# jesusbriales/dvo_slam

Hardware: AMD Instinct MI355X
Metric: frame-pairs/s (640x480, 4-level GN align) (higher is better)
Workload: dtype f32

## Files before the change

### dvo_slam_amd/capi.py

```python
from __future__ import annotations

import ctypes as C
import os

import numpy as np

from . import _build

MAX_LEVELS = 8
TERMINATION = {0: "IterationsExceeded", 1: "IncrementTooSmall", 2: "LogLikelihoodDecreased", 3: "TooFewConstraints",
               -1: "Unset"}

EXPORTS = [
    "dvo_amd_abi_version", "dvo_amd_build_id", "dvo_amd_status_string", "dvo_amd_last_error", "dvo_amd_device_count",
    "dvo_amd_default_config", "dvo_amd_context_create", "dvo_amd_context_destroy", "dvo_amd_configure",
    "dvo_amd_get_config", "dvo_amd_pyramid_create", "dvo_amd_pyramid_create_from_device", "dvo_amd_pyramid_retain",
    "dvo_amd_pyramid_release", "dvo_amd_pyramid_levels", "dvo_amd_pyramid_timestamp", "dvo_amd_pyramid_level_info",
    "dvo_amd_pyramid_download_plane", "dvo_amd_pyramid_select", "dvo_amd_match", "dvo_amd_match_batch",
    "dvo_amd_residuals", "dvo_amd_error_image", "dvo_amd_kernel_timing", "dvo_amd_se3_exp", "dvo_amd_se3_log",
    "dvo_amd_solve6", "dvo_amd_bench_residual_pass", "dvo_amd_match_many",
    "dvo_amd_debug_finalize_stamps", "dvo_amd_comm_unique_id", "dvo_amd_comm_create", "dvo_amd_comm_destroy",
    "dvo_amd_match_sharded", "dvo_amd_match_banded", "dvo_amd_context_device", "dvo_amd_debug_combine_bands", "dvo_amd_debug_wire_layout", "dvo_amd_debug_take_wire", "dvo_amd_pyramid_create_raw",
    "dvo_amd_default_validator_stages", "dvo_amd_proposals_for_candidates", "dvo_amd_validate_proposals",
    "dvo_amd_track_frame", "dvo_amd_png_info", "dvo_amd_png_read_bgr8", "dvo_amd_png_read_gray16",
    "dvo_amd_format_trajectory_line", "dvo_amd_debug_tick_log", "dvo_amd_debug_iteration", "dvo_amd_match_selection", "dvo_amd_bench_residual_pass_pairs",
    "dvo_amd_exchange_create", "dvo_amd_exchange_attach", "dvo_amd_exchange_destroy",
    "dvo_amd_match_submit", "dvo_amd_match_wait", "dvo_amd_match_poll", "dvo_amd_debug_next_seq",
    "dvo_amd_set_reciprocal_mode", "dvo_amd_get_reciprocal_mode", "dvo_amd_debug_rcp", "dvo_amd_debug_block_trace",
    "dvo_amd_debug_ll_overflow", "dvo_amd_debug_marker", "dvo_amd_debug_rcp_form", "dvo_amd_debug_weights", "dvo_amd_debug_hw_queue",
    "dvo_amd_debug_level_geometry", "dvo_amd_point_cloud", "dvo_amd_map_cloud", "dvo_amd_voxel_downsample", "dvo_amd_write_pcd",
    "dvo_amd_debug_map_timing", "dvo_amd_default_graph_options", "dvo_amd_optimize_graph", "dvo_amd_graph_marginals", "dvo_amd_debug_graph_timing",
    "dvo_amd_debug_graph_system", "dvo_amd_debug_graph_system_sparse", "dvo_amd_debug_graph_symbolic",
    "dvo_amd_debug_graph_sparse_timing", "dvo_amd_optimize_graphs_batch", "dvo_amd_debug_graph_batch_records",
]


class CConfig(C.Structure):
    _fields_ = [("first_level", C.c_int), ("last_level", C.c_int), ("max_iterations_per_level", C.c_int),
                ("precision", C.c_double), ("mu", C.c_double), ("use_initial_estimate", C.c_int),
                ("intensity_derivative_threshold", C.c_float), ("depth_derivative_threshold", C.c_float),
                ("segment_geometry", C.c_int), ("reserved", C.c_int)]


GEOMETRY_THROUGHPUT, GEOMETRY_LATENCY = 0, 1


class CIterationStats(C.Structure):
    _fields_ = [("id", C.c_int), ("valid_constraints", C.c_int), ("tdist_loglik", C.c_double),
                ("tdist_mean", C.c_double * 2), ("tdist_precision", C.c_double * 4), ("prior_loglik", C.c_double),
                ("increment", C.c_double * 6), ("information", C.c_double * 36), ("has_increment", C.c_int),
                ("reserved", C.c_int), ("estimate", C.c_double * 16), ("initial", C.c_double * 16)]


class CLevelStats(C.Structure):
    _fields_ = [("id", C.c_int), ("max_valid_pixels", C.c_int), ("valid_pixels", C.c_int), ("termination", C.c_int),
                ("n_iterations", C.c_int), ("first_iteration", C.c_int)]
# ... 121 lines not shown
    L.dvo_amd_debug_weights.argtypes = [vp, vp, vp, C.c_int, fp, fp, fp, C.POINTER(CQ7Probe)]
    L.dvo_amd_kernel_timing.argtypes = [vp, C.c_int, dp, C.POINTER(C.c_longlong), C.c_int]
    L.dvo_amd_bench_residual_pass.argtypes = [vp, vp, vp, C.c_int, fp, C.c_int, C.c_int, C.c_int, dp, dp,
                                              C.POINTER(C.c_int)]
    L.dvo_amd_bench_residual_pass_pairs.argtypes = [vp, C.c_int, C.POINTER(vp), C.POINTER(vp), C.c_int, fp, C.c_int, C.c_int, dp, dp,
                                                    C.POINTER(C.c_int)]
    L.dvo_amd_debug_finalize_stamps.argtypes = [vp, C.POINTER(C.c_ulonglong)]
    L.dvo_amd_comm_unique_id.argtypes = [C.POINTER(C.c_ubyte)]
    L.dvo_amd_comm_create.argtypes = [vp, C.POINTER(C.c_ubyte), C.c_int, C.c_int]
    L.dvo_amd_comm_destroy.argtypes = [vp]
    L.dvo_amd_comm_destroy.restype = None
    L.dvo_amd_exchange_create.argtypes = [vp, C.c_int, C.c_int, C.POINTER(C.c_ubyte)]
    L.dvo_amd_exchange_attach.argtypes = [vp, C.POINTER(C.c_ubyte)]
    L.dvo_amd_exchange_destroy.argtypes = [vp]
    L.dvo_amd_exchange_destroy.restype = None
    L.dvo_amd_match_sharded.argtypes = [vp, vp, vp, dp, C.POINTER(CResult)]
    L.dvo_amd_match_banded.argtypes = [vp, vp, vp, dp, C.POINTER(CResult), C.c_int]
    L.dvo_amd_debug_combine_bands.argtypes = [C.c_int, dp, dp]
    L.dvo_amd_debug_block_trace.restype = C.c_longlong
    L.dvo_amd_debug_block_trace.argtypes = [C.c_void_p, C.POINTER(C.c_ulonglong), C.c_longlong]
    L.dvo_amd_debug_wire_layout.argtypes = [C.POINTER(C.c_int), C.POINTER(C.c_int)]
    L.dvo_amd_debug_take_wire.argtypes = [C.POINTER(C.c_uint), C.c_uint, C.c_int, C.POINTER(C.c_uint)]
    L.dvo_amd_debug_next_seq.argtypes = [C.c_uint]
    L.dvo_amd_debug_next_seq.restype = C.c_uint
    L.dvo_amd_point_cloud.argtypes = [vp, vp, C.c_int, dp, vp, C.c_int, vp]
    L.dvo_amd_map_cloud.argtypes = [vp, C.c_int, C.POINTER(vp), dp, C.POINTER(vp), C.POINTER(C.c_int), C.c_float, vp,
                                    C.c_longlong, C.POINTER(CCloudStats)]
    L.dvo_amd_voxel_downsample.argtypes = [vp, C.c_longlong, vp, C.c_float, vp, C.c_longlong, C.POINTER(CCloudStats)]
    L.dvo_amd_write_pcd.argtypes = [C.c_char_p, vp, C.c_longlong, C.c_int, C.c_int]
    L.dvo_amd_debug_map_timing.argtypes = [vp, dp, dp, C.POINTER(C.c_longlong)]
    L.dvo_amd_se3_exp.argtypes = [dp, dp]
    L.dvo_amd_se3_exp.restype = None
    L.dvo_amd_se3_log.argtypes = [dp, dp]
    L.dvo_amd_se3_log.restype = None
    L.dvo_amd_solve6.argtypes = [dp, dp, dp]
    L.dvo_amd_solve6.restype = None
    _lib = L
    return L


def build_id() -> str:
    return lib().dvo_amd_build_id().decode()


def _check(status: int, where: str):
    if status != 0:
# ... 582 lines not shown


def comm_unique_id() -> bytes:
    buf = (C.c_ubyte * 128)()
    _check(lib().dvo_amd_comm_unique_id(buf), "dvo_amd_comm_unique_id")
    return bytes(buf)


def wire_layout():
    a, b = C.c_int(), C.c_int()
    _check(lib().dvo_amd_debug_wire_layout(C.byref(a), C.byref(b)), "wire_layout")
    return a.value, b.value


def take_wire(wire: np.ndarray, tick: int, from_piece: int, record: np.ndarray) -> int:
    up = C.POINTER(C.c_uint)
    assert wire.dtype == np.uint32 and record.dtype == np.uint32 and wire.flags.c_contiguous and record.flags.c_contiguous
    rc = lib().dvo_amd_debug_take_wire(wire.ctypes.data_as(up), tick, from_piece, record.ctypes.data_as(up))
    if rc < 0:
        _check(-rc, "take_wire")
    return rc


def combine_bands(bands) -> np.ndarray:
    b = np.ascontiguousarray(bands, dtype=np.float64)
    out = np.zeros(7)
    dp = C.POINTER(C.c_double)
    _check(lib().dvo_amd_debug_combine_bands(b.shape[0], b.ctypes.data_as(dp), out.ctypes.data_as(dp)), "combine_bands")
    return out
```

### dvo_slam_amd/csrc/dvo_internal.h

```cpp
#pragma once
#include <hip/hip_runtime.h>
#include <rccl/rccl.h>

#include <atomic>
#include <deque>
#include <memory>
#include <mutex>
#include <string>
#include <vector>

#include "../../include/dvo_amd.h"
#include "../../include/dvo_amd_debug.h"
#include "dvo_types.h"
#include "se3.h"

namespace dvo_amd {
namespace host {

extern thread_local std::string g_last_error;
int fail_hip(const char *what, hipError_t e);

#define HIP_TRY(expr)                                                     \
  do {                                                                    \
    hipError_t e_ = (expr);                                               \
// ... 120 lines not shown
  unsigned *x_host_seq = nullptr;
  unsigned x_seq = 0;
  bool x_broken = false;
  ExchangeArgs *x_args_dev = nullptr;
  ncclResult_t (*p_allgather)(const void *, void *, size_t, ncclDataType_t, ncclComm_t, hipStream_t) = nullptr;
  ncclResult_t (*p_comm_destroy)(ncclComm_t) = nullptr;
  unsigned tick_seq = 0;
  RcpTable rcp = {nullptr, 0, 0, nullptr};
  unsigned *rcp_table_dev = nullptr;
  unsigned *rcp_nibbles_dev = nullptr;
  int rcp_unit = 0;
  std::string rcp_form_note;
  int q7_off256 = 0;
  float *dbg_w_dev = nullptr;
  size_t dbg_w_capacity = 0;
  unsigned *ovf_host = nullptr, *ovf_dev = nullptr;
  long long ovf_checks = 0, ovf_hits = 0;
  long long level_steps_at[5] = {18, 70, 1000, 1000, 1LL << 40};
  long long level_steps_at_latency[5] = {250, 4000, 38400, 999999, 1LL << 40};
  int fine_steps = 0;
  int fault_slot_alloc = -1;
  bool fin_stamps = false;
  bool sort_items = true;
  bool fin_priority = true;
  bool small_args = true;
  bool poll = true;
  bool timing = false;
  double timing_ms = 0.0;
  long long timing_launches = 0;
  std::vector<double> tick_log;
  std::vector<double> tick_log_pending;
  std::vector<std::pair<hipEvent_t, hipEvent_t>> events;
  size_t events_used = 0;
  host::MapWorkspace *map_ws = nullptr;
  host::GraphWorkspace *graph_ws = nullptr;
  host::GraphBatchWorkspace *graph_batch_ws = nullptr;
};

namespace dvo_amd {
namespace host {

struct IterCtx {
  int k = 0;
  int buf = 0;
  int steps = 4;
  int n_blocks = 0;
// ... 154 lines not shown
```

### dvo_slam_amd/csrc/dvo_kernels.hip

```cpp
#include <cstddef>
#include <cstdlib>
#include <cstring>
#include <mutex>
#include <vector>

#include "dvo_types.h"

namespace dvo_amd {


#define DVO_HWREG_MODE_FP32_ROUND (1 | (0 << 6) | ((2 - 1) << 11))
#define DVO_OPAQUE(x) asm volatile("" : "+v"(x))
#ifndef DVO_KT_SGPR
#define DVO_KT_SGPR 1
#endif

__device__ __forceinline__ void round_toward_zero() { __builtin_amdgcn_s_setreg(DVO_HWREG_MODE_FP32_ROUND, 3); }
__device__ __forceinline__ void round_to_nearest() { __builtin_amdgcn_s_setreg(DVO_HWREG_MODE_FP32_ROUND, 0); }

__device__ __forceinline__ float mul_legacy(float a, float b) {
  float r;
  asm("v_mul_legacy_f32 %0, %1, %2" : "=v"(r) : "v"(a), "v"(b));
  return r;
}

// ... 830 lines not shown
      unsigned hw, xcc;
      asm volatile("s_getreg_b32 %0, hwreg(HW_REG_HW_ID)" : "=s"(hw));
      asm volatile("s_getreg_b32 %0, hwreg(HW_REG_XCC_ID)" : "=s"(xcc));
      BlockTrace t;
      t.t0 = trace_t0, t.t_first = trace_first, t.t_end = trace_t1;
#ifdef DVO_TRACE_TAIL
      if (bx < rb) {
        const unsigned long long t_spin = trace_clock();
        unsigned long long tail = 0;
        while ((tail = __hip_atomic_load(&trace_tail, __ATOMIC_RELAXED, __HIP_MEMORY_SCOPE_WORKGROUP)) == 0 && trace_clock() - t_spin < 2000) {}
        t.t_first = tail;
      }
#endif
      t.info = (unsigned)(bx < rb ? (it.steps_log2 & 15) : (it.steps_log2 >> 4)) | (bx < rb ? 0u : 16u) | ((unsigned)(d.w / 8) << 8) |
               ((unsigned)(bx < rb ? rb : it.ll_blocks) << 16);
      t.hw = (hw & 0x0fffffffu) | (xcc << 28);
      g_trace[slot] = t;
    }
  }
#endif
}

template <class Args>
__device__ __forceinline__ int tick_locate(const Args &args, int &bx, const unsigned block = blockIdx.x) {
  constexpr int kSlots = (int)(sizeof(args.group_first) / sizeof(args.group_first[0]));
  if (!args.compact) {
    const int rot = args.xcd_rot[blockIdx.y];
    bx = (int)((block & ~7u) | ((block + rot) & 7u));
    return (int)blockIdx.y;
  }
  const int lane = threadIdx.x & (kWave - 1);
  const unsigned g = block >> 3;
  const unsigned first = lane <= args.n_items ? (unsigned)args.group_first[lane < kSlots ? lane : 0] : 0xFFFFFFFFu;
  const int idx = __builtin_amdgcn_readfirstlane(__popcll(__ballot(first <= g)) - 1);
  bx = (int)block - ((int)args.group_first[idx] << 3);
  bx = (bx & ~7) | ((bx + (int)args.xcd_rot[idx]) & 7);
  return idx;
}

template <int ACC, int RCP>
__global__ __launch_bounds__(kBlockThreads, ACC == 0 ? 2 : 4) void k_tick(const TickArgs args) {
  int bx;
  const int idx = tick_locate(args, bx);
  tick_body<ACC, RCP>(args.items[idx], args.rcp, bx);
}

template <int RCP>
__global__ __launch_bounds__(kBlockThreads, 4) void k_tick_small(const TickArgsSmall args) {
  int bx;
  const int idx = tick_locate(args, bx);
  tick_body<1, RCP>(args.items[idx], args.rcp, bx);
}

template <class Args>
__device__ __forceinline__ void q7_tail_wave(const Args &args) {
  const TickItem &it = args.items[blockIdx.x];
  const int lane = threadIdx.x;
  LevelPairDesc d = load_desc(it);
  d.rcp = args.rcp;
  d.rcp_lds = nullptr, d.dbg_w = nullptr;
// ... 166 lines not shown
  bool held;
  LaunchGuard() {
    held = launch_lock_enabled();
    if (held) g_launch_mu.lock();
  }
  ~LaunchGuard() {
    if (held) g_launch_mu.unlock();
  }
};

int acc_mode() {
  static const int m = [] {
    const char *a = getenv("DVO_AMD_ACCUM");
    return (a && (a[0] == 'v' || a[0] == 'V' || a[0] == '0')) ? 0 : 1;
  }();
  return m;
}

typedef void (*TickKernel)(const TickArgs);
static TickKernel pick_tick_kernel(const RcpTable &rcp) {
  return rcp.nibbles ? k_tick<1, 2> : rcp.table ? k_tick<1, 1> : acc_mode() == 0 ? k_tick<0, 0> : k_tick<1, 0>;
}

template <class Args>
static int tick_args_layout_impl(Args &args, int max_blocks) {
  constexpr int kSlots = (int)(sizeof(args.group_first) / sizeof(args.group_first[0]));
  unsigned groups = 0;
  for (int i = 0; i < args.n_items; ++i) {
    args.group_first[i] = (uint16_t)groups;
    groups += ((unsigned)args.items[i].res_blocks + args.items[i].ll_blocks + 7u) >> 3;
  }
  for (int i = args.n_items; i < kSlots; ++i) args.group_first[i] = (uint16_t)groups;
  static const bool rotate = [] {
    const char *e = getenv("DVO_AMD_XCD_ROTATE");
    return !(e && e[0] == '0');
  }();
  long long load[8] = {0, 0, 0, 0, 0, 0, 0, 0};
  for (int i = 0; i < args.n_items; ++i) {
    const TickItem &it = args.items[i];
    const int rb = it.res_blocks, lb = it.ll_blocks;
    const long long w_res = 33 + 21 * item_res_steps(it), w_ll = 40 + 7 * item_ll_steps(it);
    long long phase[8];
    for (int f = 0; f < 8; ++f) {
      const int n_res = (rb >> 3) + (f < (rb & 7) ? 1 : 0);
      const int all = ((rb + lb) >> 3) + (f < ((rb + lb) & 7) ? 1 : 0);
      phase[f] = w_res * n_res + w_ll * (all - n_res);
    }
    int best = 0;
    long long best_max = -1;
    for (int rot = 0; rotate && rot < 8; ++rot) {
      long long mx = 0;
      for (int x = 0; x < 8; ++x) mx = std::max(mx, load[x] + phase[(x + rot) & 7]);
      if (best_max < 0 || mx < best_max) best_max = mx, best = rot;
    }
    args.xcd_rot[i] = (uint8_t)best;
    for (int x = 0; x < 8; ++x) load[x] += phase[(x + best) & 7];
  }
  for (int i = args.n_items; i < (int)(sizeof(args.xcd_rot) / sizeof(args.xcd_rot[0])); ++i) args.xcd_rot[i] = 0;
  const long long grid2d = (long long)((max_blocks + 7) & ~7) * args.n_items;
  static const int mode = [] {
    const char *e = getenv("DVO_AMD_COMPACT_GRID");
    return e ? (e[0] == '0' ? 0 : 1) : 2;
  }();
  args.compact = groups > 0 && groups < 65536 && (mode == 1 || (mode == 2 && 2ll * 8 * groups < grid2d)) ? 1 : 0;
  return (int)(groups * 8);
}
int tick_args_layout(TickArgs &args, int max_blocks) { return tick_args_layout_impl(args, max_blocks); }
int tick_args_layout(TickArgsSmall &args, int max_blocks) { return tick_args_layout_impl(args, max_blocks); }

hipError_t launch_tick_small(const TickArgsSmall &args, int max_blocks, hipStream_t stream, hipEvent_t t_start, hipEvent_t t_stop) {
  if (acc_mode() != 1) return hipErrorNotSupported;
  if (args.n_items <= 0 || max_blocks <= 0) return hipSuccess;
  LaunchGuard guard;
  dim3 grid((unsigned)((max_blocks + 7) & ~7), (unsigned)args.n_items, 1);
  if (args.compact) grid = dim3((unsigned)args.group_first[args.n_items] * 8u, 1, 1);
  if (t_start && t_stop) {
    void *kargs[] = {const_cast<TickArgsSmall *>(&args)};
    const void *kernel = args.rcp.nibbles ? reinterpret_cast<const void *>(&k_tick_small<2>)
                         : args.rcp.table ? reinterpret_cast<const void *>(&k_tick_small<1>)
                                          : reinterpret_cast<const void *>(&k_tick_small<0>);
    const hipError_t e = hipExtLaunchKernel(kernel, grid, dim3(kBlockThreads), kargs, 0, stream, t_start, t_stop, 0);
    if (e != hipSuccess) return e;
  } else if (args.rcp.nibbles) {
    hipLaunchKernelGGL(k_tick_small<2>, grid, dim3(kBlockThreads), 0, stream, args);
  } else if (args.rcp.table) {
    hipLaunchKernelGGL(k_tick_small<1>, grid, dim3(kBlockThreads), 0, stream, args);
  } else {
    hipLaunchKernelGGL(k_tick_small<0>, grid, dim3(kBlockThreads), 0, stream, args);
  }
  return hipGetLastError();
}
// ... 730 lines not shown
```

### dvo_slam_amd/csrc/dvo_probes.cpp

```cpp
#include <dlfcn.h>
#include <emmintrin.h>

#include <algorithm>
#include <cfloat>
#include <chrono>
#include <cmath>
#include <cstdio>
#include <cstdlib>
#include <cstring>
#include <limits>
#include <vector>

#include "dvo_internal.h"

using namespace dvo_amd;
using namespace dvo_amd::host;

extern "C" {

int dvo_amd_debug_rcp_form(const dvo_amd_context *ctx, int *form, char *note, int note_capacity) {
  if (!ctx || !form) return DVO_AMD_ERR_INVALID_ARGUMENT;
  *form = ctx->rcp.nibbles ? 2 : ctx->rcp.table ? 1 : 0;
  if (note && note_capacity > 0) std::snprintf(note, (size_t)note_capacity, "%s", ctx->rcp_form_note.c_str());
  return DVO_AMD_OK;
// ... 16 lines not shown
  if (e == hipSuccess) e = hipStreamSynchronize(ctx->stream);
  (void)hipFree(d_in);
  (void)hipFree(d_out);
  if (e != hipSuccess) return fail_hip("dvo_amd_debug_rcp", e);
  return DVO_AMD_OK;
}

unsigned dvo_amd_debug_next_seq(unsigned seq) { return next_seq(seq); }

int dvo_amd_debug_wire_layout(int *n_pieces, int *n_record_words) {
  if (!n_pieces || !n_record_words) return DVO_AMD_ERR_INVALID_ARGUMENT;
  *n_pieces = kFinWirePieces, *n_record_words = kFinWords;
  return DVO_AMD_OK;
}

int dvo_amd_debug_take_wire(const unsigned *wire, unsigned tick, int from_piece, unsigned *record_words) {
  if (!wire || !record_words || from_piece < 0 || from_piece > kFinWirePieces || (reinterpret_cast<uintptr_t>(wire) & 15u))
    return -DVO_AMD_ERR_INVALID_ARGUMENT;
  FinOut rec;
  std::memcpy(&rec, record_words, sizeof(rec));
  const int next = take_wire(reinterpret_cast<const FinWire *>(wire), &rec, tick, from_piece);
  std::memcpy(record_words, &rec, sizeof(rec));
  return next;
}

}

namespace dvo_amd {
namespace host {

int single_tick(dvo_amd_context *ctx, dvo_amd_pyramid *reference, dvo_amd_pyramid *current, int level, const Selection *sel, const float *T,
                const float P[4], bool unit_weights, bool residual_pass, bool loglik_pass, int ll_cut_rank) {
  const LevelData &R = reference->lv[level];
  const LevelData &C = current->lv[level];
  JobSlot &s = ctx->slots[0];
  TickArgs ta;
  std::memset(&ta, 0, sizeof(ta));
  ta.n_items = 1;
  ta.rcp = ctx->rcp;
  TickItem &w = ta.items[0];
  w.ref = sel->ref_desc + level;
  w.cur = current->cur_desc + level;
  w.slot = ctx->slot_desc;
  const int steps = level_steps(ctx, R);
  item_set_steps(w, steps, steps);
  const int nb = level_blocks(sel, level, steps);
// ... 411 lines not shown
```

### dvo_slam_amd/csrc/dvo_tracker.cpp

```cpp
#include <dlfcn.h>
#include <emmintrin.h>

#include <algorithm>
#include <cfloat>
#include <chrono>
#include <cmath>
#include <cstdio>
#include <cstdlib>
#include <cstring>

#include "dvo_internal.h"

namespace dvo_amd {
namespace host {

thread_local std::string g_last_error;

int fail_hip(const char *what, hipError_t e) {
  g_last_error = std::string(what) + ": " + hipGetErrorString(e);
  return e == hipErrorOutOfMemory ? DVO_AMD_ERR_OUT_OF_MEMORY : DVO_AMD_ERR_HIP;
}

dvo_amd_iteration_stats *stats_push(Job &j) {
  dvo_amd_result *r = j.result;
// ... 557 lines not shown
    items.push_back(w);
    fin_items.push_back(f);
    j.result->n_ticks++;
  }
  if (items.empty()) return DVO_AMD_OK;

  const size_t cap = (size_t)std::min(std::max(ctx->items_per_launch, 1), kMaxItemsPerLaunch);
  const size_t n_launch = (items.size() + cap - 1) / cap;
  const size_t per = (items.size() + n_launch - 1) / n_launch;
  size_t launch_index = 0;
  for (size_t first = 0; first < items.size(); first += per, ++launch_index) {
    hipStream_t st;
    {
      int rc = tick_stream(ctx, ctx->timing ? 0 : grp.stream_first + launch_index, &st);
      if (rc) return rc;
    }
    TickArgs ta;
    const int n_here = (int)std::min(per, items.size() - first);
    ta.n_items = n_here;
    ta.compact = 0;
    ta.rcp = ctx->rcp;
    int max_blocks = 0;
    int order[kMaxItemsPerLaunch];
    for (int i = 0; i < n_here; ++i) order[i] = i;
    if (ctx->sort_items)
      std::stable_sort(order, order + n_here, [&](int a, int b) {
        const TickItem &x = items[first + (size_t)a], &y = items[first + (size_t)b];
        const int kx = x.res_blocks ? item_res_steps(x) : 0, ky = y.res_blocks ? item_res_steps(y) : 0;
        return kx > ky;
      });
    for (int i = 0; i < n_here; ++i) {
      ta.items[i] = items[first + (size_t)order[i]];
      max_blocks = std::max(max_blocks, (int)ta.items[i].res_blocks + (int)ta.items[i].ll_blocks);
    }
    size_t ev = 0;
    if (ctx->timing) {
      int rc = timing_begin(ctx, &ev);
      if (rc) return rc;
      double rb = 0, lb = 0, px = 0, res_steps = 0, ll_steps = 0;
      for (int i = 0; i < n_here; ++i) {
        rb += ta.items[i].res_blocks, lb += ta.items[i].ll_blocks;
        res_steps += (double)ta.items[i].res_blocks * kWavesPerBlock * item_res_steps(ta.items[i]);
        if (ta.items[i].ll_blocks) ll_steps += (double)ta.items[i].ll_level_blocks * kWavesPerBlock * item_ll_steps(ta.items[i]);
      }
      for (size_t ji = grp.lo, k = 0; ji < grp.hi; ++ji) {
        const Job &j = jobs[ji];
        if (j.done || !(j.sub_ll || j.sub_res)) continue;
        if (k >= first && k < first + (size_t)n_here && j.sub_res) px += j.sub_px;
        ++k;
      }
      const double rec[kTickLogFields] = {0.0, (double)n_here, rb, lb, (double)max_blocks, px, res_steps, ll_steps};
      ctx->tick_log_pending.insert(ctx->tick_log_pending.end(), rec, rec + kTickLogFields);
    }
// ... 4 lines not shown
      for (int i = 0; i < kMaxSmallItems; ++i) ts.items[i] = ta.items[i < n_here ? i : 0];
      (void)tick_args_layout(ts, max_blocks);
      const hipError_t es = launch_tick_small(ts, max_blocks, st, t0, t1);
      if (es == hipSuccess) {
        if (ctx->rcp.table) {
          Q7ArgsSmall qs;
          qs.n_items = 0, qs.q7_off256 = ctx->q7_off256, qs.rcp = ctx->rcp;
          for (int i = 0; i < n_here; ++i)
            if (fin_items[first + (size_t)order[i]].q7_off256) qs.items[qs.n_items++] = ta.items[i];
          for (int i = qs.n_items; i < kMaxSmallItems; ++i) qs.items[i] = ta.items[0];
          const hipError_t eq = launch_q7_tail_small(qs, st);
          if (eq != hipSuccess) return fail_hip("launch_q7_tail", eq);
        }
        FinArgsSmall fs;
        fs.n_items = n_here, fs.pad = ctx->fin_stamps ? 0x57A3 : 0;
        for (int i = 0; i < kMaxSmallItems; ++i) fs.items[i] = fin_items[first + (size_t)order[i < n_here ? i : 0]];
        const hipError_t ef = launch_finalize_small(fs, st);
        if (ef != hipSuccess) return fail_hip("launch_finalize", ef);
        continue;
      }
      if (es != hipErrorNotSupported) return fail_hip("launch_tick", es);
      (void)hipGetLastError();
    }
    (void)tick_args_layout(ta, max_blocks);
    hipError_t e = launch_tick(ta, max_blocks, st, t0, t1);
    if (e != hipSuccess) return fail_hip("launch_tick", e);
    static_assert(kMaxFinItems >= kMaxItemsPerLaunch, "one reduce launch per tick launch");
    if (ctx->rcp.table) {
      Q7Args qa;
      qa.n_items = 0, qa.q7_off256 = ctx->q7_off256, qa.rcp = ctx->rcp;
      for (int i = 0; i < n_here; ++i)
        if (fin_items[first + (size_t)order[i]].q7_off256) qa.items[qa.n_items++] = ta.items[i];
      for (int i = qa.n_items; i < kMaxItemsPerLaunch; ++i) qa.items[i] = ta.items[0];
      e = launch_q7_tail(qa, st);
      if (e != hipSuccess) return fail_hip("launch_q7_tail", e);
    }
    FinArgs fa;
    fa.n_items = n_here;
    fa.pad = ctx->fin_stamps ? 0x57A3 : 0;
    fa.exchange = nullptr, fa.xseq = 0, fa.pad2 = ctx->fin_priority ? kFinFlagPriority : 0u;
    for (int i = 0; i < n_here; ++i) fa.items[i] = fin_items[first + (size_t)order[i]];
    for (int i = n_here; i < kMaxFinItems; ++i) fa.items[i] = fa.items[0];
    e = launch_finalize(fa, st);
    if (e != hipSuccess) return fail_hip("launch_finalize", e);
  }
  grp.in_flight = true;
  if (ctx->host_prof) ctx->prof_submit_ns += now_ns() - t_begin, ctx->prof_ticks++, ctx->prof_job_ticks += (long long)items.size();
// ... 374 lines not shown
  if (hipGetDeviceCount(&ndev) != hipSuccess || ndev <= 0) return DVO_AMD_ERR_NO_DEVICE;
  if (device < 0 || device >= ndev || device >= kMaxDevices) return DVO_AMD_ERR_INVALID_ARGUMENT;
  dvo_amd_config c;
  dvo_amd_default_config(&c);
  if (cfg) c = *cfg;
  int rc = check_config(&c);
  if (rc) return rc;
  HIP_TRY(hipSetDevice(device));
  dvo_amd_context *ctx = new dvo_amd_context();
  ctx->device = device;
  ctx->cfg = c;
  hipError_t e = hipStreamCreateWithFlags(&ctx->stream, hipStreamNonBlocking);
  if (e != hipSuccess) {
    delete ctx;
    return fail_hip("hipStreamCreate", e);
  }
  const char *pe = getenv("DVO_AMD_POLL");
  ctx->poll = !(pe && pe[0] == '0');
  const char *fs = getenv("DVO_AMD_FIN_STAMPS");
  ctx->fin_stamps = fs && fs[0] == '1';
  const char *fp = getenv("DVO_AMD_FIN_PRIORITY");
  ctx->fin_priority = !(fp && fp[0] == '0');
  if (const char *so = getenv("DVO_AMD_SORT_ITEMS")) ctx->sort_items = so[0] != '0';
  const char *sa = getenv("DVO_AMD_SMALL_ARGS");
  ctx->small_args = !(sa && sa[0] == '0');
  const char *hp = getenv("DVO_AMD_HOST_PROF");
  ctx->host_prof = hp && hp[0] == '1';
  if (const char *sl = getenv("DVO_AMD_SPEC_LEVELS")) ctx->spec_levels = sl[0] == '1' ? 1 : 0;
  if (const char *fs2 = getenv("DVO_AMD_FAULT_SLOT_ALLOC")) ctx->fault_slot_alloc = atoi(fs2);
  if (const char *sa = getenv("DVO_AMD_LEVEL_STEPS_AT"))
    (void)sscanf(sa, "%lld,%lld,%lld,%lld,%lld", &ctx->level_steps_at[0], &ctx->level_steps_at[1], &ctx->level_steps_at[2],
                 &ctx->level_steps_at[3], &ctx->level_steps_at[4]);
  if (const char *fsx = getenv("DVO_AMD_FINE_STEPS")) ctx->fine_steps = atoi(fsx);
  if (const char *lm = getenv("DVO_AMD_LL_MERGE")) {
    const int v = atoi(lm);
    if (v == 1 || v == 2 || v == 4 || v == 8 || v == 16) ctx->ll_merge = v;
  }
  if (const char *rm = getenv("DVO_AMD_RCP"))
    if (rm[0] == 'h' || rm[0] == 'H' || rm[0] == 's' || rm[0] == 'S') {
      const int rrc = dvo_amd_set_reciprocal_mode(ctx, DVO_AMD_RCP_HOST_SSE);
      if (rrc) {
        dvo_amd_context_destroy(ctx);
        return rrc;
      }
    }
  if (const char *ipl = getenv("DVO_AMD_ITEMS_PER_LAUNCH")) {
// ... 290 lines not shown
```

### dvo_slam_amd/csrc/dvo_types.h

```cpp
#pragma once
#include <hip/hip_runtime.h>
#include <stdint.h>

namespace dvo_amd {

constexpr int kWave = 64;
constexpr int kBlockThreads = 256;
constexpr int kWavesPerBlock = kBlockThreads / kWave;
constexpr int kStepPx = kWave;
constexpr int kMaxSteps = 64;
constexpr int kPlanePad = kStepPx * kMaxSteps * kWavesPerBlock;

constexpr int kRecCount = 0, kRecFirstW = 1, kRecLastR = 2, kRecS0 = 4, kRecS1 = 7, kRecWaveCnt = 10, kRecAcc = 16;
constexpr int kNumAcc = 87;
constexpr int kRecStride = 104;
constexpr int kAccAA = 0, kAccAB = 21, kAccBB = 42, kAccAR0 = 63, kAccAR1 = 69, kAccBR0 = 75, kAccBR1 = 81;

constexpr int kLevelChunksMax = 16;
__host__ __device__ inline int level_chunks_log2(int nb) { return nb >= 128 ? 4 : nb >= 64 ? 3 : nb >= 32 ? 2 : nb >= 16 ? 1 : 0; }
__host__ __device__ inline int chunk_lo(int nb, int c) { return (nb * c) >> level_chunks_log2(nb); }
__host__ __device__ inline void leaf_range(int nb, int g_log2, int i, int *lo, int *hi) {
  const int per = g_log2 - level_chunks_log2(nb);
  const int c = i >> per, q = i & ((1 << per) - 1);
  const int c_lo = chunk_lo(nb, c), len = chunk_lo(nb, c + 1) - c_lo;
// ... 96 lines not shown
struct RcpTable {
  const unsigned *table;
  int shift;
  int unit;
  const unsigned *nibbles;
};
struct Q7Rec {
  double S[3];
  double acc[87];
  int n_tail, valid;
  int idx[3];
  float w_table[3];
  float w_exact[3];
  int recomputed_equal;
};
static_assert(sizeof(Q7Rec) == 768, "Q7Rec: three 256-byte lines of the slot's block");
constexpr int kRcpNibbleWordsMax = 512;
struct TickArgs {
  int n_items;
  int compact;
  RcpTable rcp;
  uint16_t group_first[kMaxItemsPerLaunch + 4];
  uint8_t xcd_rot[kMaxItemsPerLaunch + 2] = {};
  TickItem items[kMaxItemsPerLaunch];
};
static_assert(sizeof(TickArgs) <= 8192, "kernel argument block too large");

struct FinOut {
  int valid;
  int has_res;
  int has_ll;
  unsigned seq;
  double S[3];
  double S_odd[3];
  float first_w, last_r0, last_r1;
  float ll_qmax;
  double acc[kNumAcc];
  double ll_sum;
};
static_assert(sizeof(FinOut) % 16 == 0, "FinOut is copied in 16-byte pieces");

constexpr int kFinWords = (int)(sizeof(FinOut) / 4);
constexpr int kFinWirePieces = (kFinWords + 1) / 2;
struct alignas(16) FinWire {
  unsigned piece[kFinWirePieces][4];
};
// ... 34 lines not shown
  const struct ExchangeArgs *exchange;
  unsigned xseq;
  unsigned pad2;
  FinItem items[kMaxFinItems];
};
static_assert(sizeof(FinArgs) <= 4096, "kernel argument block too large");

template <int N>
struct Q7ArgsT {
  int n_items;
  int q7_off256;
  RcpTable rcp;
  TickItem items[N];
};
typedef Q7ArgsT<kMaxItemsPerLaunch> Q7Args;

constexpr int kMaxSmallItems = 8;
struct TickArgsSmall {
  int n_items;
  int compact;
  RcpTable rcp;
  uint16_t group_first[kMaxSmallItems + 4];
  uint8_t xcd_rot[kMaxSmallItems] = {};
  TickItem items[kMaxSmallItems];
};
struct FinArgsSmall {
  int n_items;
  int pad;
  FinItem items[kMaxSmallItems];
};

hipError_t launch_tick(const TickArgs &args, int max_blocks, hipStream_t stream, hipEvent_t t_start = nullptr,
                       hipEvent_t t_stop = nullptr);
int tick_args_layout(TickArgs &args, int max_blocks);
int tick_args_layout(TickArgsSmall &args, int max_blocks);
hipError_t launch_tick_small(const TickArgsSmall &args, int max_blocks, hipStream_t stream, hipEvent_t t_start = nullptr,
                             hipEvent_t t_stop = nullptr);
hipError_t launch_finalize_small(const FinArgsSmall &args, hipStream_t stream);
typedef Q7ArgsT<kMaxSmallItems> Q7ArgsSmall;
hipError_t launch_q7_tail(const Q7Args &args, hipStream_t stream);
hipError_t launch_q7_tail_small(const Q7ArgsSmall &args, hipStream_t stream);
hipError_t launch_finalize(const FinArgs &args, hipStream_t stream);
hipError_t launch_ll_overflow(const float2 *res, const int *seg_prefix, int seg_first, int n_segs, int seg_px, int rank_offset,
                              int n_px, int cut_rank, int rank_end, const float P[4], unsigned *result_host, hipStream_t stream);
hipError_t launch_exchange_record(const FinOut *rec_dev, const struct ExchangeArgs *exchange_dev, unsigned xseq, hipStream_t stream);
constexpr float kLlOverflowScreen = 7.0e6f;
hipError_t read_finalize_stamps(unsigned long long out[8]);
long long read_block_trace(unsigned long long *out, long long capacity);
hipError_t launch_rcp_table_probe(const RcpTable &rcp, const float *in, float *out, int n, hipStream_t stream);
hipError_t launch_rcp_midpoint_probe(int k, unsigned *out_rn, unsigned *out_rtz, hipStream_t stream);

hipError_t launch_marker(unsigned tag, hipStream_t stream);
hipError_t launch_queue_probe(unsigned *out_pinned, hipStream_t stream);
int acc_mode();

hipError_t launch_pyr_down(const float *i_prev, const float *z_prev, int w_prev, float *i_out, float *z_out, int w, int h,
                           hipStream_t stream);
hipError_t launch_level_planes(const float *i_plane, const float *z_plane, int w, int h, int n_pad, float fx, float fy,
// ... 15 lines not shown
```

### include/dvo_amd_debug.h

```cpp
#ifndef DVO_AMD_DEBUG_H_
#define DVO_AMD_DEBUG_H_

#include "dvo_amd.h"

#ifdef __cplusplus
extern "C" {
#endif

long long dvo_amd_debug_block_trace(dvo_amd_context *ctx, unsigned long long *out, long long capacity_blocks);
int dvo_amd_debug_rcp(dvo_amd_context *ctx, int n, const float *in, float *out);

int dvo_amd_debug_combine_bands(int n_bands, const double *bands, double *out);
unsigned dvo_amd_debug_next_seq(unsigned seq);
int dvo_amd_debug_wire_layout(int *n_pieces, int *n_record_words);
int dvo_amd_debug_take_wire(const unsigned *wire, unsigned tick, int from_piece, unsigned *record_words);

typedef struct {
  int valid_constraints;
  int reserved;
  double scale_sums[3];
  float scale[4];
  float precision[4];
  double moments[87];
  double information[36];
  double rhs[6];
  double loglik_sum;
  float loglik;
  float reserved_f;
} dvo_amd_iteration_probe;
int dvo_amd_debug_iteration(dvo_amd_context *ctx, dvo_amd_pyramid *reference, dvo_amd_pyramid *current, int level,
                            const float *T, const float *precision_in, const float *precision_eval,
                            dvo_amd_iteration_probe *out);

typedef struct {
  int n_tail;
  int valid_constraints;
  int valid_counted;
  int recomputed_equal;
// ... 59 lines not shown
```

Before: 61740.

## Group tick items sharing a reference into sets for joint XCD placement

Items that share the same reference level and block geometry are sorted next to each other and treated as a set when choosing XCD rotations. The default share mode of 1 rotates each set as a unit so its blocks land on the same XCDs and can reuse the reference data in L2. A tail rebalance step is also added for when per-XCD load becomes uneven. An optional mode 2 interleaves the blocks of a set, which costs a division per block inside the kernel. The added placement logic and per-item arrays make the kernel argument block larger, and the gain only appears when batches actually contain items that share a reference.

```diff
diff --git a/dvo_slam_amd/capi.py b/dvo_slam_amd/capi.py
--- a/dvo_slam_amd/capi.py
+++ b/dvo_slam_amd/capi.py
@@ -32,6 +32,7 @@
     "dvo_amd_debug_map_timing", "dvo_amd_default_graph_options", "dvo_amd_optimize_graph", "dvo_amd_graph_marginals", "dvo_amd_debug_graph_timing",
     "dvo_amd_debug_graph_system", "dvo_amd_debug_graph_system_sparse", "dvo_amd_debug_graph_symbolic",
     "dvo_amd_debug_graph_sparse_timing", "dvo_amd_optimize_graphs_batch", "dvo_amd_debug_graph_batch_records",
+    "dvo_amd_debug_tick_layout",
 ]
 
 
@@ -199,6 +200,8 @@
     L.dvo_amd_debug_wire_layout.argtypes = [C.POINTER(C.c_int), C.POINTER(C.c_int)]
     L.dvo_amd_debug_take_wire.argtypes = [C.POINTER(C.c_uint), C.c_uint, C.c_int, C.POINTER(C.c_uint)]
     L.dvo_amd_debug_next_seq.argtypes = [C.c_uint]
+    ip = C.POINTER(C.c_int)
+    L.dvo_amd_debug_tick_layout.argtypes = [C.c_int, ip, ip, ip, ip, ip, C.c_int, C.c_int, ip, ip, ip, ip, ip, ip, ip, C.c_longlong, ip, ip]
     L.dvo_amd_debug_next_seq.restype = C.c_uint
     L.dvo_amd_point_cloud.argtypes = [vp, vp, C.c_int, dp, vp, C.c_int, vp]
     L.dvo_amd_map_cloud.argtypes = [vp, C.c_int, C.POINTER(vp), dp, C.POINTER(vp), C.POINTER(C.c_int), C.c_float, vp,
@@ -827,6 +830,24 @@
     return rc
 
 
+def tick_layout(res_blocks, ll_blocks, res_steps, ref_key, cur_key, share: int, max_blocks: int = 0) -> dict:
+    ip = C.POINTER(C.c_int)
+    ins = [np.ascontiguousarray(a, np.int32) for a in (res_blocks, ll_blocks, res_steps, ref_key, cur_key)]
+    n = len(ins[0])
+    assert all(len(a) == n for a in ins)
+    order, rot, tail, size = (np.zeros(n, np.int32) for _ in range(4))
+    first = np.zeros(n + 1, np.int32)
+    compact, n_blocks = C.c_int(), C.c_int()
+    cap = 8 * 65536
+    b_item, b_index = np.full(cap, -2, np.int32), np.full(cap, -2, np.int32)
+    p = lambda a: a.ctypes.data_as(ip)
+    _check(lib().dvo_amd_debug_tick_layout(n, *[p(a) for a in ins], share, max_blocks, p(order), p(first), p(rot), p(tail), p(size),
+                                           C.byref(compact), C.byref(n_blocks), cap, p(b_item), p(b_index)), "tick_layout")
+    nb = n_blocks.value if compact.value else 0
+    return dict(order=order, group_first=first, xcd_rot=rot, tail_rot=tail, set_size=size, compact=compact.value,
+                n_blocks=n_blocks.value, block_item=b_item[:nb], block_index=b_index[:nb])
+
+
 def combine_bands(bands) -> np.ndarray:
     b = np.ascontiguousarray(bands, dtype=np.float64)
     out = np.zeros(7)
diff --git a/dvo_slam_amd/csrc/dvo_internal.h b/dvo_slam_amd/csrc/dvo_internal.h
--- a/dvo_slam_amd/csrc/dvo_internal.h
+++ b/dvo_slam_amd/csrc/dvo_internal.h
@@ -166,6 +166,7 @@
   int fault_slot_alloc = -1;
   bool fin_stamps = false;
   bool sort_items = true;
+  int share_placement = 1;
   bool fin_priority = true;
   bool small_args = true;
   bool poll = true;
diff --git a/dvo_slam_amd/csrc/dvo_kernels.hip b/dvo_slam_amd/csrc/dvo_kernels.hip
--- a/dvo_slam_amd/csrc/dvo_kernels.hip
+++ b/dvo_slam_amd/csrc/dvo_kernels.hip
@@ -1,6 +1,8 @@
+#include <algorithm>
 #include <cstddef>
 #include <cstdlib>
 #include <cstring>
+#include <functional>
 #include <mutex>
 #include <vector>
 
@@ -877,20 +879,31 @@
 }
 
 template <class Args>
+__host__ __device__ __forceinline__ int tick_place(const Args &args, int idx, int pos, const unsigned block, int &bx) {
+  if constexpr (Args::kSets) {
+    if (args.compact > 1) {
+      const unsigned m = args.set_size[idx];
+      if (m > 1) {
+        const unsigned q = (unsigned)(((unsigned long long)(unsigned)pos * args.set_inv[idx]) >> 32);
+        idx += pos - (int)(q * m);
+        pos = (int)q;
+      }
+    }
+  }
+  const int rot = pos < (int)(args.items[idx].res_blocks >> 3) ? args.xcd_rot[idx] : args.tail_rot[idx];
+  bx = (pos << 3) | (int)((block + (unsigned)rot) & 7u);
+  return idx;
+}
+
+template <class Args>
 __device__ __forceinline__ int tick_locate(const Args &args, int &bx, const unsigned block = blockIdx.x) {
   constexpr int kSlots = (int)(sizeof(args.group_first) / sizeof(args.group_first[0]));
-  if (!args.compact) {
-    const int rot = args.xcd_rot[blockIdx.y];
-    bx = (int)((block & ~7u) | ((block + rot) & 7u));
-    return (int)blockIdx.y;
-  }
+  if (!args.compact) return tick_place(args, (int)blockIdx.y, (int)(block >> 3), block, bx);
   const int lane = threadIdx.x & (kWave - 1);
   const unsigned g = block >> 3;
   const unsigned first = lane <= args.n_items ? (unsigned)args.group_first[lane < kSlots ? lane : 0] : 0xFFFFFFFFu;
   const int idx = __builtin_amdgcn_readfirstlane(__popcll(__ballot(first <= g)) - 1);
-  bx = (int)block - ((int)args.group_first[idx] << 3);
-  bx = (bx & ~7) | ((bx + (int)args.xcd_rot[idx]) & 7);
-  return idx;
+  return tick_place(args, idx, (int)g - (int)args.group_first[idx], block, bx);
 }
 
 template <int ACC, int RCP>
@@ -1103,51 +1116,138 @@
   return rcp.nibbles ? k_tick<1, 2> : rcp.table ? k_tick<1, 1> : acc_mode() == 0 ? k_tick<0, 0> : k_tick<1, 0>;
 }
 
+static bool same_set(const TickItem &a, const TickItem &b) {
+  return a.res_blocks > 0 && a.ref == b.ref && a.res_blocks == b.res_blocks && a.res_first == b.res_first &&
+         (a.steps_log2 & 15) == (b.steps_log2 & 15);
+}
+static int layout_tail_mode() {
+  static const int m = [] {
+    const char *e = getenv("DVO_AMD_SHARE_TAIL");
+    return e ? (e[0] == '0' ? 0 : 1) : 2;
+  }();
+  return m;
+}
 template <class Args>
-static int tick_args_layout_impl(Args &args, int max_blocks) {
+static int tick_args_layout_impl(Args &args, int max_blocks, int share) {
   constexpr int kSlots = (int)(sizeof(args.group_first) / sizeof(args.group_first[0]));
-  unsigned groups = 0;
-  for (int i = 0; i < args.n_items; ++i) {
-    args.group_first[i] = (uint16_t)groups;
-    groups += ((unsigned)args.items[i].res_blocks + args.items[i].ll_blocks + 7u) >> 3;
-  }
-  for (int i = args.n_items; i < kSlots; ++i) args.group_first[i] = (uint16_t)groups;
+  constexpr int kRots = (int)(sizeof(args.xcd_rot) / sizeof(args.xcd_rot[0]));
+  const int n = args.n_items;
+  if constexpr (!Args::kSets) share = 0;
   static const bool rotate = [] {
     const char *e = getenv("DVO_AMD_XCD_ROTATE");
     return !(e && e[0] == '0');
   }();
-  long long load[8] = {0, 0, 0, 0, 0, 0, 0, 0};
-  for (int i = 0; i < args.n_items; ++i) {
+  int set_len[kRots] = {};
+  bool any_set = false;
+  for (int i = 0; i < n;) {
+    int j = i + 1;
+    while (share > 0 && j < n && same_set(args.items[i], args.items[j])) ++j;
+    set_len[i] = j - i;
+    any_set = any_set || j - i > 1;
+    i = j;
+  }
+  long long phase[kRots][8];
+  for (int i = 0; i < n; ++i) {
     const TickItem &it = args.items[i];
     const int rb = it.res_blocks, lb = it.ll_blocks;
     const long long w_res = 33 + 21 * item_res_steps(it), w_ll = 40 + 7 * item_ll_steps(it);
-    long long phase[8];
     for (int f = 0; f < 8; ++f) {
       const int n_res = (rb >> 3) + (f < (rb & 7) ? 1 : 0);
       const int all = ((rb + lb) >> 3) + (f < ((rb + lb) & 7) ? 1 : 0);
-      phase[f] = w_res * n_res + w_ll * (all - n_res);
-    }
-    int best = 0;
-    long long best_max = -1;
-    for (int rot = 0; rotate && rot < 8; ++rot) {
-      long long mx = 0;
-      for (int x = 0; x < 8; ++x) mx = std::max(mx, load[x] + phase[(x + rot) & 7]);
-      if (best_max < 0 || mx < best_max) best_max = mx, best = rot;
-    }
-    args.xcd_rot[i] = (uint8_t)best;
-    for (int x = 0; x < 8; ++x) load[x] += phase[(x + best) & 7];
-  }
-  for (int i = args.n_items; i < (int)(sizeof(args.xcd_rot) / sizeof(args.xcd_rot[0])); ++i) args.xcd_rot[i] = 0;
+      phase[i][f] = w_res * n_res + w_ll * (all - n_res);
+    }
+  }
+  long long load[8];
+  auto balance = [&](bool by_set, uint8_t *rot_out) {
+    for (int x = 0; x < 8; ++x) load[x] = 0;
+    for (int i = 0; i < n;) {
+      const int len = by_set ? set_len[i] : 1;
+      long long ph[8] = {0, 0, 0, 0, 0, 0, 0, 0};
+      for (int k = i; k < i + len; ++k)
+        for (int f = 0; f < 8; ++f) ph[f] += phase[k][f];
+      int best = 0;
+      long long best_max = -1;
+      for (int rot = 0; rotate && rot < 8; ++rot) {
+        long long mx = 0;
+        for (int x = 0; x < 8; ++x) mx = std::max(mx, load[x] + ph[(x + rot) & 7]);
+        if (best_max < 0 || mx < best_max) best_max = mx, best = rot;
+      }
+      for (int k = i; k < i + len; ++k) rot_out[k] = (uint8_t)best;
+      for (int x = 0; x < 8; ++x) load[x] += ph[(x + best) & 7];
+      i += len;
+    }
+  };
+  balance(true, args.xcd_rot);
+  for (int i = 0; i < n; ++i) args.tail_rot[i] = args.xcd_rot[i];
+  if (any_set && rotate) {
+    long long lo = load[0], hi = load[0], sum = 0;
+    for (int x = 0; x < 8; ++x) lo = std::min(lo, load[x]), hi = std::max(hi, load[x]), sum += load[x];
+    const int tail_mode = layout_tail_mode();
+    if (tail_mode == 1 || (tail_mode == 2 && (hi - lo) * 8 * 50 > sum)) {
+      balance(false, args.tail_rot);
+      for (int i = 0; i < n; ++i) args.xcd_rot[i] = 0;
+    }
+  }
+  for (int i = n; i < kRots; ++i) args.xcd_rot[i] = args.tail_rot[i] = 0;
+
+  const bool interleave = share > 1 && any_set;
+  unsigned groups = 0;
+  auto item_groups = [&](int i) { return ((unsigned)args.items[i].res_blocks + args.items[i].ll_blocks + 7u) >> 3; };
+  for (int i = 0; i < n;) {
+    const int len = interleave ? set_len[i] : 1;
+    unsigned widest = 0;
+    for (int k = i; k < i + len; ++k) widest = std::max(widest, item_groups(k));
+    args.group_first[i] = (uint16_t)groups;
+    groups += (unsigned)len * widest;
+    for (int k = i + 1; k < i + len; ++k) args.group_first[k] = (uint16_t)groups;
+    if constexpr (Args::kSets) {
+      for (int k = i; k < i + len; ++k) args.set_size[k] = 1, args.set_inv[k] = 0;
+      if (len > 1) args.set_size[i] = (uint8_t)len, args.set_inv[i] = (uint32_t)(0xFFFFFFFFull / (unsigned)len + 1ull);
+    }
+    i += len;
+  }
+  for (int i = n; i < kSlots; ++i) args.group_first[i] = (uint16_t)groups;
+  if constexpr (Args::kSets)
+    for (int i = n; i < kRots; ++i) args.set_size[i] = 1;
   const long long grid2d = (long long)((max_blocks + 7) & ~7) * args.n_items;
   static const int mode = [] {
     const char *e = getenv("DVO_AMD_COMPACT_GRID");
     return e ? (e[0] == '0' ? 0 : 1) : 2;
   }();
-  args.compact = groups > 0 && groups < 65536 && (mode == 1 || (mode == 2 && 2ll * 8 * groups < grid2d)) ? 1 : 0;
+  unsigned own_groups = 0;
+  for (int i = 0; i < n; ++i) own_groups += item_groups(i);
+  args.compact = groups > 0 && groups < 65536 && (mode == 1 || (mode == 2 && 2ll * 8 * own_groups < grid2d)) ? (interleave ? 2 : 1) : 0;
+  if (!args.compact && share > 0) return tick_args_layout_impl(args, max_blocks, 0);
   return (int)(groups * 8);
 }
-int tick_args_layout(TickArgs &args, int max_blocks) { return tick_args_layout_impl(args, max_blocks); }
-int tick_args_layout(TickArgsSmall &args, int max_blocks) { return tick_args_layout_impl(args, max_blocks); }
+int tick_args_layout(TickArgs &args, int max_blocks, int share) { return tick_args_layout_impl(args, max_blocks, share); }
+int tick_args_layout(TickArgsSmall &args, int max_blocks) { return tick_args_layout_impl(args, max_blocks, 0); }
+
+void tick_items_order(const TickItem *items, int n, bool sort, int share, int *order) {
+  for (int i = 0; i < n; ++i) order[i] = i;
+  if (!sort) return;
+  std::stable_sort(order, order + n, [&](int a, int b) {
+    const TickItem &x = items[a], &y = items[b];
+    const int kx = x.res_blocks ? item_res_steps(x) : 0, ky = y.res_blocks ? item_res_steps(y) : 0;
+    if (kx != ky || share <= 0) return kx > ky;
+    if (x.ref != y.ref) return std::less<const void *>()(x.ref, y.ref);
+    return std::less<const void *>()(x.cur, y.cur);
+  });
+}
+
+int tick_args_locate(const TickArgs &args, unsigned block, int *bx) {
+  *bx = -1;
+  if (!args.compact || (block >> 3) >= (unsigned)args.group_first[args.n_items]) return -1;
+  int idx = -1;
+  for (int i = 0; i <= args.n_items; ++i)
+    if ((unsigned)args.group_first[i] <= (block >> 3)) idx = i;
+  if (idx < 0 || idx >= args.n_items) return -1;
+  int b;
+  idx = tick_place(args, idx, (int)(block >> 3) - (int)args.group_first[idx], block, b);
+  if (idx >= args.n_items || b >= (int)args.items[idx].res_blocks + (int)args.items[idx].ll_blocks) return -1;
+  *bx = b;
+  return idx;
+}
 
 hipError_t launch_tick_small(const TickArgsSmall &args, int max_blocks, hipStream_t stream, hipEvent_t t_start, hipEvent_t t_stop) {
   if (acc_mode() != 1) return hipErrorNotSupported;
diff --git a/dvo_slam_amd/csrc/dvo_probes.cpp b/dvo_slam_amd/csrc/dvo_probes.cpp
--- a/dvo_slam_amd/csrc/dvo_probes.cpp
+++ b/dvo_slam_amd/csrc/dvo_probes.cpp
@@ -62,6 +62,44 @@
   const int next = take_wire(reinterpret_cast<const FinWire *>(wire), &rec, tick, from_piece);
   std::memcpy(record_words, &rec, sizeof(rec));
   return next;
+}
+
+int dvo_amd_debug_tick_layout(int n_items, const int *res_blocks, const int *ll_blocks, const int *res_steps, const int *ref_key,
+                              const int *cur_key, int share, int max_blocks, int *order, int *group_first, int *xcd_rot,
+                              int *tail_rot, int *set_size, int *compact, int *n_blocks, long long capacity_blocks, int *block_item,
+                              int *block_index) {
+  if (n_items < 1 || n_items > kMaxItemsPerLaunch || !res_blocks || !ll_blocks || !res_steps || !ref_key || !cur_key || !order ||
+      !group_first || !xcd_rot || !tail_rot || !set_size || !compact || !n_blocks || share < 0 || share > 2 || !block_item != !block_index)
+    return DVO_AMD_ERR_INVALID_ARGUMENT;
+  std::vector<TickItem> items((size_t)n_items);
+  int widest = 0;
+  for (int i = 0; i < n_items; ++i) {
+    TickItem &w = items[(size_t)i];
+    std::memset(&w, 0, sizeof(w));
+    if (res_blocks[i] < 0 || res_blocks[i] > 2048 || ll_blocks[i] < 0 || ll_blocks[i] > 2048 || ref_key[i] < 0 || cur_key[i] < 0)
+      return DVO_AMD_ERR_INVALID_ARGUMENT;
+    w.ref = reinterpret_cast<const RefLevelDesc *>(uintptr_t(4096) + sizeof(RefLevelDesc) * (size_t)ref_key[i]);
+    w.cur = reinterpret_cast<const CurLevelDesc *>(uintptr_t(4096) + sizeof(CurLevelDesc) * (size_t)cur_key[i]);
+    w.res_blocks = (uint16_t)res_blocks[i], w.ll_blocks = (uint16_t)ll_blocks[i];
+    item_set_steps(w, res_steps[i], res_steps[i]);
+    if (item_res_steps(w) != res_steps[i]) return DVO_AMD_ERR_INVALID_ARGUMENT;
+    widest = std::max(widest, res_blocks[i] + ll_blocks[i]);
+  }
+  tick_items_order(items.data(), n_items, true, share, order);
+  TickArgs ta;
+  ta.n_items = n_items, ta.compact = 0;
+  std::memset(&ta.rcp, 0, sizeof(ta.rcp));
+  for (int k = 0; k < n_items; ++k) ta.items[k] = items[(size_t)order[k]];
+  *n_blocks = tick_args_layout(ta, max_blocks > 0 ? max_blocks : widest, share);
+  *compact = ta.compact ? 1 : 0;
+  for (int k = 0; k < n_items; ++k)
+    group_first[k] = ta.group_first[k], xcd_rot[k] = ta.xcd_rot[k], tail_rot[k] = ta.tail_rot[k], set_size[k] = ta.set_size[k];
+  group_first[n_items] = ta.group_first[n_items];
+  if (block_item && ta.compact) {
+    if (capacity_blocks < (long long)*n_blocks) return DVO_AMD_ERR_INVALID_ARGUMENT;
+    for (int b = 0; b < *n_blocks; ++b) block_item[b] = tick_args_locate(ta, (unsigned)b, &block_index[b]);
+  }
+  return DVO_AMD_OK;
 }
 
 }
diff --git a/dvo_slam_amd/csrc/dvo_tracker.cpp b/dvo_slam_amd/csrc/dvo_tracker.cpp
--- a/dvo_slam_amd/csrc/dvo_tracker.cpp
+++ b/dvo_slam_amd/csrc/dvo_tracker.cpp
@@ -603,13 +603,7 @@
     ta.rcp = ctx->rcp;
     int max_blocks = 0;
     int order[kMaxItemsPerLaunch];
-    for (int i = 0; i < n_here; ++i) order[i] = i;
-    if (ctx->sort_items)
-      std::stable_sort(order, order + n_here, [&](int a, int b) {
-        const TickItem &x = items[first + (size_t)a], &y = items[first + (size_t)b];
-        const int kx = x.res_blocks ? item_res_steps(x) : 0, ky = y.res_blocks ? item_res_steps(y) : 0;
-        return kx > ky;
-      });
+    tick_items_order(items.data() + first, n_here, ctx->sort_items, ctx->share_placement, order);
     for (int i = 0; i < n_here; ++i) {
       ta.items[i] = items[first + (size_t)order[i]];
       max_blocks = std::max(max_blocks, (int)ta.items[i].res_blocks + (int)ta.items[i].ll_blocks);
@@ -660,7 +654,7 @@
       if (es != hipErrorNotSupported) return fail_hip("launch_tick", es);
       (void)hipGetLastError();
     }
-    (void)tick_args_layout(ta, max_blocks);
+    (void)tick_args_layout(ta, max_blocks, ctx->share_placement);
     hipError_t e = launch_tick(ta, max_blocks, st, t0, t1);
     if (e != hipSuccess) return fail_hip("launch_tick", e);
     static_assert(kMaxFinItems >= kMaxItemsPerLaunch, "one reduce launch per tick launch");
@@ -1081,6 +1075,7 @@
   const char *fp = getenv("DVO_AMD_FIN_PRIORITY");
   ctx->fin_priority = !(fp && fp[0] == '0');
   if (const char *so = getenv("DVO_AMD_SORT_ITEMS")) ctx->sort_items = so[0] != '0';
+  if (const char *sp = getenv("DVO_AMD_SHARE_PLACEMENT")) ctx->share_placement = sp[0] == '0' ? 0 : sp[0] == '2' ? 2 : 1;
   const char *sa = getenv("DVO_AMD_SMALL_ARGS");
   ctx->small_args = !(sa && sa[0] == '0');
   const char *hp = getenv("DVO_AMD_HOST_PROF");
diff --git a/dvo_slam_amd/csrc/dvo_types.h b/dvo_slam_amd/csrc/dvo_types.h
--- a/dvo_slam_amd/csrc/dvo_types.h
+++ b/dvo_slam_amd/csrc/dvo_types.h
@@ -142,6 +142,10 @@
   RcpTable rcp;
   uint16_t group_first[kMaxItemsPerLaunch + 4];
   uint8_t xcd_rot[kMaxItemsPerLaunch + 2] = {};
+  uint8_t tail_rot[kMaxItemsPerLaunch + 2] = {};
+  uint8_t set_size[kMaxItemsPerLaunch + 2] = {};
+  uint32_t set_inv[kMaxItemsPerLaunch] = {};
+  static constexpr bool kSets = true;
   TickItem items[kMaxItemsPerLaunch];
 };
 static_assert(sizeof(TickArgs) <= 8192, "kernel argument block too large");
@@ -222,6 +226,8 @@
   RcpTable rcp;
   uint16_t group_first[kMaxSmallItems + 4];
   uint8_t xcd_rot[kMaxSmallItems] = {};
+  uint8_t tail_rot[kMaxSmallItems] = {};
+  static constexpr bool kSets = false;
   TickItem items[kMaxSmallItems];
 };
 struct FinArgsSmall {
@@ -232,8 +238,10 @@
 
 hipError_t launch_tick(const TickArgs &args, int max_blocks, hipStream_t stream, hipEvent_t t_start = nullptr,
                        hipEvent_t t_stop = nullptr);
-int tick_args_layout(TickArgs &args, int max_blocks);
+int tick_args_layout(TickArgs &args, int max_blocks, int share = 0);
 int tick_args_layout(TickArgsSmall &args, int max_blocks);
+void tick_items_order(const TickItem *items, int n, bool sort, int share, int *order);
+int tick_args_locate(const TickArgs &args, unsigned block, int *bx);
 hipError_t launch_tick_small(const TickArgsSmall &args, int max_blocks, hipStream_t stream, hipEvent_t t_start = nullptr,
                              hipEvent_t t_stop = nullptr);
 hipError_t launch_finalize_small(const FinArgsSmall &args, hipStream_t stream);
diff --git a/include/dvo_amd_debug.h b/include/dvo_amd_debug.h
--- a/include/dvo_amd_debug.h
+++ b/include/dvo_amd_debug.h
@@ -14,6 +14,10 @@
 unsigned dvo_amd_debug_next_seq(unsigned seq);
 int dvo_amd_debug_wire_layout(int *n_pieces, int *n_record_words);
 int dvo_amd_debug_take_wire(const unsigned *wire, unsigned tick, int from_piece, unsigned *record_words);
+int dvo_amd_debug_tick_layout(int n_items, const int *res_blocks, const int *ll_blocks, const int *res_steps, const int *ref_key,
+                              const int *cur_key, int share, int max_blocks, int *order, int *group_first, int *xcd_rot,
+                              int *tail_rot, int *set_size, int *compact, int *n_blocks, long long capacity_blocks, int *block_item,
+                              int *block_index);
 
 typedef struct {
   int valid_constraints;
```

Result: faster. 62800, median of 6 (+1.7%).
